# neuronika/neuronika

Measured on NVIDIA H100. Metric: forward+backward GFLOP/s, higher is better.
Workload: dtype bf16

## Files before the change

neuronika_b200/csrc/nk_gemm_tc.cu:

```cuda
#include "nk_internal.cuh"
#include "nk_ptx.cuh"

namespace {

constexpr int BLOCK_M = 128;
constexpr int BLOCK_K = 64;
constexpr int WGMMA_K = 16;
constexpr int kNumThreads = 384;
constexpr uint32_t kSmemLimit = 232448;
constexpr int kEpiCols = 64;
constexpr uint32_t kEpiStageBytes = 2 * 64 * kEpiCols * 4;

struct GemmParams {
  int64_t M, N, K;
  int64_t ldc;
  void* C;
  const void* bias;
  float alpha, beta;
  int bias_bf16;
  int bias_per_row;
  int relu;
  const void* mask;
  float* colsum;
  int num_m_blocks, num_n_blocks, num_k_blocks;
  uint32_t a_lbo, a_sbo, a_kstep;
  uint32_t b_lbo, b_sbo, b_kstep;
  int rs_world, m_rot;
  int64_t rs_rows;
  void* rs_dst[8];
  int batch, a_batched, b_batched, batch_reduce, splits;
  int64_t c_batch_stride;
  int tma_store;
  int64_t bias_batch_stride;
};

__device__ __forceinline__ int tile_m_block(const GemmParams& p, int tile) {
  const int t = tile % p.num_m_blocks;
  if (p.rs_world == 0) return t;
  const int owner = (t + p.m_rot) % p.rs_world;
  return owner * (p.num_m_blocks / p.rs_world) + t / p.rs_world;
}

constexpr int kGroupM = 16;
__device__ __forceinline__ void tile_coords(const GemmParams& p, int tile, int& m_blk, int& n_blk) {
  if (p.rs_world) {
    m_blk = tile_m_block(p, tile);
    n_blk = tile / p.num_m_blocks;
    return;
  }
  const int group_size = kGroupM * p.num_n_blocks;
  const int group = tile / group_size, in_group = tile - group * group_size;
  const int first_m = group * kGroupM;
  const int gm = min(p.num_m_blocks - first_m, kGroupM);
  m_blk = first_m + in_group % gm;
  n_blk = in_group / gm;
}

template <int BLOCK_N>
struct Cfg {
  static constexpr uint32_t A_BYTES = BLOCK_M * BLOCK_K * 2;
  static constexpr uint32_t B_BYTES = BLOCK_N * BLOCK_K * 2;
  static constexpr uint32_t STAGE_BYTES = A_BYTES + B_BYTES;
  static constexpr int kStagesMax = (kSmemLimit - 2048 - kEpiStageBytes) / STAGE_BYTES;
  static constexpr int kStages = kStagesMax > 8 ? 8 : kStagesMax;
  static constexpr uint32_t SMEM_BYTES = kStages * STAGE_BYTES + 2048 + kEpiStageBytes;
};

__device__ __forceinline__ void scale_and_bias(const GemmParams& p, const void* bias, int64_t row, int64_t col0,
                                               const uint32_t* r, bool full, float* v) {
#pragma unroll
  for (int j = 0; j < 32; ++j) v[j] = __fmul_rn(p.alpha, __uint_as_float(r[j]));
  if (bias && p.bias_per_row) {
    const float b = p.bias_bf16 ? __bfloat162float(static_cast<const __nv_bfloat16*>(bias)[row]) : static_cast<const float*>(bias)[row];
#pragma unroll
    for (int j = 0; j < 32; ++j) v[j] += b;
  } else if (bias) {
    if (full && (reinterpret_cast<uintptr_t>(bias) & 15) == 0) {
      if (p.bias_bf16) {
        const uint4* bp = reinterpret_cast<const uint4*>(static_cast<const __nv_bfloat16*>(bias) + col0);
#pragma unroll
        for (int q = 0; q < 4; ++q) {
          const uint4 w = __ldg(bp + q);
          const uint32_t ww[4] = {w.x, w.y, w.z, w.w};
#pragma unroll
          for (int i = 0; i < 4; ++i) {
            v[q * 8 + 2 * i] += __uint_as_float(ww[i] << 16);
            v[q * 8 + 2 * i + 1] += __uint_as_float(ww[i] & 0xffff0000u);
          }
        }
      } else {
        const float4* bp = reinterpret_cast<const float4*>(static_cast<const float*>(bias) + col0);
#pragma unroll
        for (int q = 0; q < 8; ++q) {
          const float4 w = __ldg(bp + q);
          v[q * 4] += w.x, v[q * 4 + 1] += w.y, v[q * 4 + 2] += w.z, v[q * 4 + 3] += w.w;
        }
      }
    } else {
#pragma unroll
      for (int j = 0; j < 32; ++j)
        if (col0 + j < p.N)
          v[j] += p.bias_bf16 ? __bfloat162float(static_cast<const __nv_bfloat16*>(bias)[col0 + j])
                              : static_cast<const float*>(bias)[col0 + j];
    }
  }
}

template <typename TC>
__device__ __forceinline__ void epilogue_colsum_chunk32(const GemmParams& p, int64_t row, int64_t col0, const uint32_t* r,
                                                        int lane, bool vec_ok) {
  float v[32];
  const bool live = row < p.M;
  const TC* mrow = (p.mask && live) ? static_cast<const TC*>(p.mask) + row * p.ldc + col0 : nullptr;
  const bool full = col0 + 32 <= p.N;
#pragma unroll
  for (int j = 0; j < 32; ++j) v[j] = (live && col0 + j < p.N) ? p.alpha * __uint_as_float(r[j]) : 0.f;
  if (mrow) {
    if (full && vec_ok) {
// ... 56 lines not shown
    constexpr int V = 16 / sizeof(TC);
    if (mrow) {
#pragma unroll
      for (int q = 0; q < 32 / V; ++q) {
        NkVec<TC> mk;
        mk.load(mrow + q * V);
#pragma unroll
        for (int i = 0; i < V; ++i) v[q * V + i] = mk.get(i) > 0.f ? v[q * V + i] : 0.f;
      }
    }
    if (p.beta != 0.f) {
#pragma unroll
      for (int q = 0; q < 32 / V; ++q) {
        NkVec<TC> c;
        c.load(crow + q * V);
#pragma unroll
        for (int i = 0; i < V; ++i) v[q * V + i] += p.beta * c.get(i);
      }
    }
    if (p.relu) {
#pragma unroll
      for (int j = 0; j < 32; ++j) v[j] = v[j] > 0.f ? v[j] : 0.f;
    }
#pragma unroll
    for (int q = 0; q < 32 / V; ++q) {
      NkVec<TC> o;
#pragma unroll
      for (int i = 0; i < V; ++i) o.set(i, v[q * V + i]);
      o.store(crow + q * V);
    }
  } else {
#pragma unroll
    for (int j = 0; j < 32; ++j) {
      if (j < ncols && col0 + j < p.N) {
        float x = v[j];
        if (mrow) x = nk_to_f32<TC>(mrow[j]) > 0.f ? x : 0.f;
        if (p.beta != 0.f) x += p.beta * nk_to_f32<TC>(crow[j]);
        if (p.relu) x = x > 0.f ? x : 0.f;
        crow[j] = nk_from_f32<TC>(x);
      }
    }
  }
}

__device__ __forceinline__ int epi_index(int row, int col) {
  return row * kEpiCols + ((((col >> 2) ^ (row & 7))) << 2) + (col & 3);
}

__device__ __forceinline__ float col_bias(const GemmParams& p, int64_t col) {
  if (col >= p.N) return 0.f;
  return p.bias_bf16 ? __bfloat162float(static_cast<const __nv_bfloat16*>(p.bias)[col]) : static_cast<const float*>(p.bias)[col];
}

__device__ __forceinline__ float epi_value(const GemmParams& p, float acc, float bias) {
  float v = __fmul_rn(p.alpha, acc);
  if (p.bias) v += bias;
  return p.relu ? (v > 0.f ? v : 0.f) : v;
}

template <int BLOCK_N, bool A_MN, bool B_MN, typename TC, bool BATCH = false, bool BATCH_BIAS = false>
__global__ void __launch_bounds__(kNumThreads, 1)
gemm_tc_kernel(const __grid_constant__ CUtensorMap tmap_a, const __grid_constant__ CUtensorMap tmap_b,
               const __grid_constant__ CUtensorMap tmap_c, const GemmParams p) {
  using C_ = Cfg<BLOCK_N>;
  constexpr int kStages = C_::kStages;
  constexpr int kStoreCols = 128 / int(sizeof(TC));
  constexpr bool kTmaStore = !BATCH && BLOCK_N % kStoreCols == 0;
  static_assert(2 * 2 * 64 * 128 <= kEpiStageBytes, "staging buffers");
  extern __shared__ uint8_t smem_raw[];
  const uint32_t smem_base = (ptx::smem_u32(smem_raw) + 1023u) & ~1023u;
  const uint32_t smem_a0 = smem_base;
  const uint32_t smem_b0 = smem_base + kStages * C_::A_BYTES;
  const uint32_t bar_base = smem_base + kStages * C_::STAGE_BYTES;
  auto full_bar = [&](int s) { return bar_base + 8u * s; };
  auto empty_bar = [&](int s) { return bar_base + 8u * (kStages + s); };
  const uint32_t epi_stage = bar_base + 1024;
  float* epi = reinterpret_cast<float*>(smem_raw + (epi_stage - ptx::smem_u32(smem_raw)));

  const int wg = threadIdx.x >> 7;
  const int lane = threadIdx.x & 31;

  if (threadIdx.x == 0) {
    ptx::prefetch_tmap(&tmap_a);
    ptx::prefetch_tmap(&tmap_b);
    if (kTmaStore && p.tma_store) ptx::prefetch_tmap(&tmap_c);
    for (int s = 0; s < kStages; ++s) {
      ptx::mbar_init(full_bar(s), 1);
      ptx::mbar_init(empty_bar(s), 2);
    }
    ptx::fence_barrier_init();
  }
  __syncthreads();

  const int tiles_mn = p.num_m_blocks * p.num_n_blocks;
  const int num_tiles = BATCH ? tiles_mn * (p.batch_reduce ? p.splits : p.batch) : tiles_mn;
  auto batch_range = [&](int outer, int& b0, int& b1) {
    if (!p.batch_reduce) {
      b0 = outer, b1 = outer + 1;
    } else {
      const int per = (p.batch + p.splits - 1) / p.splits;
      b0 = outer * per;
      b1 = min(p.batch, b0 + per);
    }
  };

  if (wg == 0) {
    ptx::setmaxnreg_dec<40>();
    if (threadIdx.x == 0) {
      int stage = 0;
      uint32_t phase = 0;
      for (int tile = blockIdx.x; tile < num_tiles; tile += gridDim.x) {
        int m_blk, n_blk, b0 = 0, b1 = 1;
        tile_coords(p, BATCH ? tile % tiles_mn : tile, m_blk, n_blk);
        if (BATCH) batch_range(tile / tiles_mn, b0, b1);
        const int m0 = m_blk * BLOCK_M, n0 = n_blk * BLOCK_N;
        for (int bb = b0; bb < b1; ++bb)
        for (int kb = 0; kb < p.num_k_blocks; ++kb) {
          ptx::mbar_wait_spin(empty_bar(stage), phase ^ 1u);
          ptx::mbar_expect_tx(full_bar(stage), C_::STAGE_BYTES);
          const int k0 = kb * BLOCK_K;
          const uint32_t sa = smem_a0 + stage * C_::A_BYTES;
          const uint32_t sb = smem_b0 + stage * C_::B_BYTES;
          if (A_MN) {
#pragma unroll
            for (int c = 0; c < BLOCK_M / 64; ++c) {
              if (BATCH && p.a_batched)
                ptx::tma_load_3d(sa + c * (64 * BLOCK_K * 2), &tmap_a, full_bar(stage), m0 + c * 64, k0, bb);
              else
                ptx::tma_load_2d(sa + c * (64 * BLOCK_K * 2), &tmap_a, full_bar(stage), m0 + c * 64, k0);
            }
          } else {
            if (BATCH && p.a_batched)
              ptx::tma_load_3d(sa, &tmap_a, full_bar(stage), k0, m0, bb);
            else
              ptx::tma_load_2d(sa, &tmap_a, full_bar(stage), k0, m0);
          }
          if (B_MN) {
#pragma unroll
            for (int c = 0; c < BLOCK_N / 64; ++c) {
              if (BATCH && p.b_batched)
                ptx::tma_load_3d(sb + c * (64 * BLOCK_K * 2), &tmap_b, full_bar(stage), n0 + c * 64, k0, bb);
              else
                ptx::tma_load_2d(sb + c * (64 * BLOCK_K * 2), &tmap_b, full_bar(stage), n0 + c * 64, k0);
            }
          } else {
            if (BATCH && p.b_batched)
              ptx::tma_load_3d(sb, &tmap_b, full_bar(stage), k0, n0, bb);
            else
              ptx::tma_load_2d(sb, &tmap_b, full_bar(stage), k0, n0);
          }
          if (++stage == kStages) {
            stage = 0;
            phase ^= 1u;
          }
        }
      }
    }
    return;
  }

  ptx::setmaxnreg_inc<232>();
  const int cw = wg - 1;
  const int t = threadIdx.x & 127;
  const int warp = t >> 5;
  const bool vec_ok = ((p.ldc * int64_t(sizeof(TC))) % 16 == 0) && ((reinterpret_cast<uintptr_t>(p.C) & 15) == 0) &&
                      ((reinterpret_cast<uintptr_t>(p.mask) & 15) == 0);
  float* stg = epi + cw * (64 * kEpiCols);
  const uint32_t a_off = uint32_t(cw) * (64 * BLOCK_K * 2);
  float acc[BLOCK_N / 2];
  int stage = 0;
  uint32_t phase = 0;
  uint32_t store_buf = 0;
  for (int tile = blockIdx.x; tile < num_tiles; tile += gridDim.x) {
    int m_blk, n_blk;
    tile_coords(p, BATCH ? tile % tiles_mn : tile, m_blk, n_blk);
    int k_total = p.num_k_blocks;
    if (BATCH) {
      int b0, b1;
      batch_range(tile / tiles_mn, b0, b1);
      k_total *= (b1 - b0);
    }
    int prev_stage = 0;
    for (int kb = 0; kb < k_total; ++kb) {
      ptx::mbar_wait_spin(full_bar(stage), phase);
      const uint64_t adesc = ptx::make_smem_desc_sw128(smem_a0 + stage * C_::A_BYTES + a_off, p.a_lbo, p.a_sbo);
      const uint64_t bdesc = ptx::make_smem_desc_sw128(smem_b0 + stage * C_::B_BYTES, p.b_lbo, p.b_sbo);
      ptx::fence_regs(acc);
      ptx::wgmma_fence();
#pragma unroll
      for (int k = 0; k < BLOCK_K / WGMMA_K; ++k)
        ptx::Wgmma<BLOCK_N>::template mma<int(A_MN), int(B_MN)>(acc, adesc + uint64_t((k * p.a_kstep) >> 4),
                                                                 bdesc + uint64_t((k * p.b_kstep) >> 4), (kb | k) != 0 ? 1u : 0u);
      ptx::wgmma_commit();
      ptx::wgmma_wait<1>();
      ptx::fence_regs(acc);
      if (kb > 0 && t == 0) ptx::mbar_arrive(empty_bar(prev_stage));
      prev_stage = stage;
      if (++stage == kStages) {
        stage = 0;
        phase ^= 1u;
      }
    }
    ptx::wgmma_wait<0>();
    ptx::fence_regs(acc);
    if (t == 0) ptx::mbar_arrive(empty_bar(prev_stage));

    if constexpr (kTmaStore) {
      if (p.tma_store) {
        const int fr = warp * 16 + (lane >> 2);
        const int q = lane & 3;
        const int row0 = m_blk * BLOCK_M + cw * 64;
        const uint32_t stg0 = epi_stage + uint32_t(cw) * (2 * 64 * 128);
#pragma unroll
        for (int ch = 0; ch < BLOCK_N / kStoreCols; ++ch) {
          const uint32_t buf = stg0 + store_buf * (64 * 128);
          if (t == 0) ptx::tma_store_wait_read<1>();
          ptx::named_barrier(1 + cw, 128);
          const int64_t col0 = int64_t(n_blk) * BLOCK_N + ch * kStoreCols;
#pragma unroll
          for (int jj = 0; jj < kStoreCols / 8; ++jj) {
            const int j = (ch * (kStoreCols / 8) + jj) * 4;
            const int64_t col = col0 + jj * 8 + 2 * q;
            float b0 = 0.f, b1 = 0.f;
            if (p.bias) b0 = col_bias(p, col), b1 = col_bias(p, col + 1);
            const float v0 = epi_value(p, acc[j], b0), v1 = epi_value(p, acc[j + 1], b1);
            const float v2 = epi_value(p, acc[j + 2], b0), v3 = epi_value(p, acc[j + 3], b1);
            if constexpr (sizeof(TC) == 2) {
              const uint32_t off = fr * 128 + ((jj ^ (fr & 7)) << 4) + 4 * q;
              const __nv_bfloat162 lo = __floats2bfloat162_rn(v0, v1), hi = __floats2bfloat162_rn(v2, v3);
              ptx::st_shared_b32(buf + off, *reinterpret_cast<const uint32_t*>(&lo));
              ptx::st_shared_b32(buf + off + 8 * 128, *reinterpret_cast<const uint32_t*>(&hi));
            } else {
              const uint32_t off = fr * 128 + (((2 * jj + (q >> 1)) ^ (fr & 7)) << 4) + (q & 1) * 8;
              ptx::st_shared_v2_f32(buf + off, v0, v1);
              ptx::st_shared_v2_f32(buf + off + 8 * 128, v2, v3);
            }
          }
          ptx::fence_proxy_async();
          ptx::named_barrier(1 + cw, 128);
          if (t == 0) {
            if (row0 < p.M && col0 < p.N) ptx::tma_store_2d(&tmap_c, buf, int(col0), row0);
            ptx::tma_store_commit();
          }
          store_buf ^= 1u;
        }
        continue;
      }
    }

    const int64_t c_off = (BATCH && !p.batch_reduce) ? int64_t(tile / tiles_mn) * p.c_batch_stride : 0;
    const bool atomic = BATCH && p.batch_reduce;
    const int fr = warp * 16 + (lane >> 2);
    const int fc = (lane & 3) * 2;
    const int half = warp >> 1;
    const int rloc = (warp & 1) * 32 + lane;
    const int64_t row = int64_t(m_blk) * BLOCK_M + cw * 64 + rloc;
    constexpr int kChunks = (BLOCK_N + kEpiCols - 1) / kEpiCols;
#pragma unroll
    for (int ch = 0; ch < kChunks; ++ch) {
      constexpr int kFullBlocks = kEpiCols / 8;
      ptx::named_barrier(1 + cw, 128);
#pragma unroll
      for (int nb = 0; nb < kFullBlocks; ++nb) {
        if (ch * kFullBlocks + nb < BLOCK_N / 8) {
          const int j = (ch * kFullBlocks + nb) * 4;
          *reinterpret_cast<float2*>(stg + epi_index(fr, nb * 8 + fc)) = make_float2(acc[j], acc[j + 1]);
          *reinterpret_cast<float2*>(stg + epi_index(fr + 8, nb * 8 + fc)) = make_float2(acc[j + 2], acc[j + 3]);
        }
      }
      ptx::named_barrier(1 + cw, 128);
      const int chunk_cols = BLOCK_N - ch * kEpiCols < kEpiCols ? BLOCK_N - ch * kEpiCols : kEpiCols;
      if (!vec_ok && !p.colsum && !p.mask && !p.rs_world) {
        const int64_t col_base = int64_t(n_blk) * BLOCK_N + ch * kEpiCols;
        for (int rr = 0; rr < 16; ++rr) {
          const int srow = warp * 16 + rr;
          const int64_t grow = int64_t(m_blk) * BLOCK_M + cw * 64 + srow;
          if (grow >= p.M) break;
          const void* bias = p.bias;
          if constexpr (BATCH_BIAS) bias = batch_bias<true>(p, c_off);
          float rb = 0.f;
          if (bias && p.bias_per_row)
            rb = p.bias_bf16 ? __bfloat162float(static_cast<const __nv_bfloat16*>(bias)[grow]) : static_cast<const float*>(bias)[grow];
          for (int c = lane; c < chunk_cols; c += 32) {
            const int64_t col = col_base + c;
            if (col >= p.N) break;
            float v = __fmul_rn(p.alpha, stg[epi_index(srow, c)]);
            TC* cp = static_cast<TC*>(p.C) + c_off + grow * p.ldc + col;
            if (atomic) {
              if constexpr (sizeof(TC) == 4) atomicAdd(reinterpret_cast<float*>(cp), v);
              continue;
            }
            if (bias) {
              v += p.bias_per_row ? rb
                                  : (p.bias_bf16 ? __bfloat162float(static_cast<const __nv_bfloat16*>(bias)[col])
                                                 : static_cast<const float*>(bias)[col]);
            }
            if (p.beta != 0.f) v += p.beta * nk_to_f32<TC>(*cp);
            if (p.relu) v = v > 0.f ? v : 0.f;
            *cp = nk_from_f32<TC>(v);
          }
        }
        continue;
      }
      const int ncols = min(32, chunk_cols - half * 32);
      if (ncols > 0) {
        uint32_t r[32];
#pragma unroll
        for (int q = 0; q < 8; ++q) {
          float4 v = make_float4(0.f, 0.f, 0.f, 0.f);
          if (q * 4 < ncols) v = *reinterpret_cast<const float4*>(stg + epi_index(rloc, half * 32 + q * 4));
          r[4 * q] = __float_as_uint(v.x), r[4 * q + 1] = __float_as_uint(v.y);
          r[4 * q + 2] = __float_as_uint(v.z), r[4 * q + 3] = __float_as_uint(v.w);
        }
        const int64_t col0 = int64_t(n_blk) * BLOCK_N + ch * kEpiCols + half * 32;
        if (p.colsum && col0 < p.N) epilogue_colsum_chunk32<TC>(p, row, col0, r, lane, vec_ok);
        if (row < p.M && col0 < p.N) epilogue_store_chunk32<TC, BATCH_BIAS>(p, row, col0, r, ncols, vec_ok, c_off, atomic);
      }
    }
  }
  if (kTmaStore && p.tma_store && t == 0) ptx::tma_store_wait<0>();
}

typedef CUresult (*EncodeTiledFn)(CUtensorMap*, CUtensorMapDataType, cuuint32_t, void*, const cuuint64_t*,
                                  const cuuint64_t*, const cuuint32_t*, const cuuint32_t*, CUtensorMapInterleave,
                                  CUtensorMapSwizzle, CUtensorMapL2promotion, CUtensorMapFloatOOBfill);

int make_tmap_2d(nk_ctx* ctx, CUtensorMap* tm, const void* base, int64_t rows, int64_t cols, int64_t ld,
                 uint32_t box_cols, uint32_t box_rows, int dtype = NK_BF16) {
  if (!ctx->encode_tiled) return nk_set_error(ctx, NK_ERR_CUDA, "cuTensorMapEncodeTiled unavailable");
  cuuint64_t dims[2] = {(cuuint64_t)cols, (cuuint64_t)rows};
  cuuint64_t strides[1] = {(cuuint64_t)ld * nk_dtype_size(dtype)};
  cuuint32_t box[2] = {box_cols, box_rows};
  cuuint32_t estr[2] = {1, 1};
  CUresult r = reinterpret_cast<EncodeTiledFn>(ctx->encode_tiled)(
      tm, dtype == NK_BF16 ? CU_TENSOR_MAP_DATA_TYPE_BFLOAT16 : CU_TENSOR_MAP_DATA_TYPE_FLOAT32, 2,
      const_cast<void*>(base), dims, strides, box, estr,
      CU_TENSOR_MAP_INTERLEAVE_NONE, CU_TENSOR_MAP_SWIZZLE_128B, CU_TENSOR_MAP_L2_PROMOTION_L2_256B,
      CU_TENSOR_MAP_FLOAT_OOB_FILL_NONE);
  if (r != CUDA_SUCCESS)
    return nk_set_error(ctx, NK_ERR_CUDA, "cuTensorMapEncodeTiled failed (%d) rows=%lld cols=%lld ld=%lld", (int)r,
                        (long long)rows, (long long)cols, (long long)ld);
  return NK_OK;
}

template <int BLOCK_N, bool A_MN, bool B_MN, typename TC, bool BATCH = false, bool BATCH_BIAS = false>
int launch_cfg(nk_ctx* ctx, const CUtensorMap& ta, const CUtensorMap& tb, const CUtensorMap& tc, GemmParams& p) {
  using C_ = Cfg<BLOCK_N>;
  auto kern = gemm_tc_kernel<BLOCK_N, A_MN, B_MN, TC, BATCH, BATCH_BIAS>;
  static bool attr_done[64] = {};
  if (!attr_done[ctx->device & 63]) {
    static_assert(C_::SMEM_BYTES <= kSmemLimit, "shared memory budget");
    NK_CUDA(ctx, cudaFuncSetAttribute(kern, cudaFuncAttributeMaxDynamicSharedMemorySize, (int)C_::SMEM_BYTES));
    attr_done[ctx->device & 63] = true;
  }
  p.num_n_blocks = int((p.N + BLOCK_N - 1) / BLOCK_N);
  int num_tiles = p.num_m_blocks * p.num_n_blocks;
  if (BATCH) {
    if (p.batch_reduce) {
      int want = (ctx->sm_count + num_tiles - 1) / num_tiles;
      if (want > p.batch) want = p.batch;
      const int per = (p.batch + want - 1) / want;
      p.splits = (p.batch + per - 1) / per;
      num_tiles *= p.splits;
    } else {
      num_tiles *= p.batch;
    }
  }
  const int units = ctx->sm_count;
  const int waves = (num_tiles + units - 1) / units;
  const int grid = (num_tiles + waves - 1) / waves;
  const size_t smem = C_::SMEM_BYTES;
  if (p.rs_world) {
    if (BLOCK_N != 256 || sizeof(TC) != 4 || p.N % 4 != 0)
// ... 60 lines not shown
  p.K = K;
  p.ldc = ldc;
  p.C = C;
  p.bias = bias;
  p.alpha = alpha;
  p.beta = beta;
  p.bias_bf16 = bias_dtype == NK_BF16;
  p.bias_per_row = 0;
  p.relu = relu;
  p.mask = mask;
  p.colsum = colsum;
  p.batch = 1, p.a_batched = p.b_batched = p.batch_reduce = 0, p.splits = 1, p.c_batch_stride = 0, p.bias_batch_stride = 0;
  p.num_m_blocks = int((M + BLOCK_M - 1) / BLOCK_M);
  p.num_n_blocks = 0;
  p.num_k_blocks = int((K + BLOCK_K - 1) / BLOCK_K);
  p.rs_world = 0;
  p.m_rot = 0;
  p.rs_rows = M;
  for (int i = 0; i < 8; ++i) p.rs_dst[i] = nullptr;
  if (ctx->rs_world > 1) {
    if (M % (int64_t(ctx->rs_world) * BLOCK_M) != 0 || beta != 0.f || c_dtype != NK_F32)
      return nk_set_error(ctx, NK_ERR_INVALID_ARG, "wgmma gemm: reduce-scatter epilogue needs M %% (world*128) == 0, "
                          "beta == 0 and f32 output");
    p.rs_world = ctx->rs_world;
    p.rs_rows = M / ctx->rs_world;
    p.m_rot = ctx->rs_rank;
    for (int i = 0; i < ctx->rs_world; ++i) p.rs_dst[i] = ctx->rs_dst[i];
  }
  p.a_lbo = a_mn ? BLOCK_K * 128 : 16;
  p.a_sbo = 1024;
  p.a_kstep = a_mn ? WGMMA_K * 128 : WGMMA_K * 2;
  p.b_lbo = b_mn ? BLOCK_K * 128 : 16;
  p.b_sbo = 1024;
  p.b_kstep = b_mn ? WGMMA_K * 128 : WGMMA_K * 2;

  CUtensorMap ta, tb;
  int rc;
  if (a_mn)
    rc = make_tmap_2d(ctx, &ta, A, K, M, lda, 64, BLOCK_K);
  else
    rc = make_tmap_2d(ctx, &ta, A, M, K, lda, BLOCK_K, BLOCK_M);
  if (rc) return rc;
  if (b_mn)
    rc = make_tmap_2d(ctx, &tb, B, K, N, ldb, 64, BLOCK_K);
  else
    rc = make_tmap_2d(ctx, &tb, B, N, K, ldb, BLOCK_K, (uint32_t)block_n);
  if (rc) return rc;
  const int64_t c_size = int64_t(nk_dtype_size(c_dtype));
  CUtensorMap tc;
  memset(&tc, 0, sizeof(tc));
  p.tma_store = beta == 0.f && !mask && !colsum && !p.rs_world && (block_n * c_size) % 128 == 0 &&
                (reinterpret_cast<uintptr_t>(C) & 15) == 0 && (ldc * c_size) % 16 == 0 && (N * c_size) % 16 == 0;
  if (p.tma_store) {
    rc = make_tmap_2d(ctx, &tc, C, M, N, ldc, uint32_t(128 / c_size), 64, c_dtype);
    if (rc) return rc;
  }

  static const char* names[2][2][5] = {
      {{"wgmma_nt_128x256", "wgmma_nt_128x128", "wgmma_nt_128x64", "wgmma_nt_128x32", "wgmma_nt_128x16"},
       {"wgmma_nn_128x256", "wgmma_nn_128x128", "wgmma_nn_128x64", "", ""}},
      {{"wgmma_tt_128x256", "wgmma_tt_128x128", "wgmma_tt_128x64", "wgmma_tt_128x32", "wgmma_tt_128x16"},
       {"wgmma_tn_128x256", "wgmma_tn_128x128", "wgmma_tn_128x64", "", ""}}};
  const int bi = block_n == 256 ? 0 : block_n == 128 ? 1 : block_n == 64 ? 2 : block_n == 32 ? 3 : 4;
  ctx->last_gemm_kernel = names[a_mn][b_mn][bi];

#define NK_TC(AM, BM_)                                                              \
  (c_dtype == NK_BF16 ? launch_bn<AM, BM_, __nv_bfloat16>(ctx, block_n, ta, tb, tc, p) \
                      : launch_bn<AM, BM_, float>(ctx, block_n, ta, tb, tc, p))
  if (!a_mn && !b_mn) return NK_TC(false, false);
  if (!a_mn && b_mn) return NK_TC(false, true);
  if (a_mn && !b_mn) return NK_TC(true, false);
  return NK_TC(true, true);
#undef NK_TC
}

static int make_tmap_3d(nk_ctx* ctx, CUtensorMap* tm, const void* base, int64_t rows, int64_t cols, int64_t ld, int64_t batch,
                        int64_t batch_stride, uint32_t box_cols, uint32_t box_rows) {
  if (!ctx->encode_tiled) return nk_set_error(ctx, NK_ERR_CUDA, "cuTensorMapEncodeTiled unavailable");
  cuuint64_t dims[3] = {(cuuint64_t)cols, (cuuint64_t)rows, (cuuint64_t)batch};
  cuuint64_t strides[2] = {(cuuint64_t)ld * 2, (cuuint64_t)batch_stride * 2};
  cuuint32_t box[3] = {box_cols, box_rows, 1};
  cuuint32_t estr[3] = {1, 1, 1};
  CUresult r = reinterpret_cast<EncodeTiledFn>(ctx->encode_tiled)(
      tm, CU_TENSOR_MAP_DATA_TYPE_BFLOAT16, 3, const_cast<void*>(base), dims, strides, box, estr,
      CU_TENSOR_MAP_INTERLEAVE_NONE, CU_TENSOR_MAP_SWIZZLE_128B, CU_TENSOR_MAP_L2_PROMOTION_L2_256B,
      CU_TENSOR_MAP_FLOAT_OOB_FILL_NONE);
  if (r != CUDA_SUCCESS)
    return nk_set_error(ctx, NK_ERR_CUDA, "cuTensorMapEncodeTiled (3-d) failed (%d) rows=%lld cols=%lld ld=%lld batch=%lld stride=%lld",
                        (int)r, (long long)rows, (long long)cols, (long long)ld, (long long)batch, (long long)batch_stride);
  return NK_OK;
}

static int gemm_wgmma_batched(nk_ctx* ctx, int transA, int transB, int64_t M, int64_t N, int64_t K, float alpha, const void* A,
                              int64_t lda, int64_t strideA, const void* B, int64_t ldb, int64_t strideB, float beta, void* C,
                              int64_t ldc, int64_t strideC, int64_t batch, int c_dtype, const void* bias, int bias_dtype,
                              int bias_per_row, int64_t bias_stride, int relu, int reduce) {
  if (!nk_gemm_wgmma_supported(transA, transB, M, N, K, A, lda, B, ldb)) return NK_ERR_UNSUPPORTED;
  if (batch < 1 || batch > (int64_t(1) << 30) || (strideA * 2) % 16 != 0 || (strideB * 2) % 16 != 0) return NK_ERR_UNSUPPORTED;
  if (reduce && c_dtype != NK_F32) return NK_ERR_UNSUPPORTED;
  const bool a_mn = transA != 0, b_mn = transB == 0;
  int block_n = N <= 64 ? 64 : (N <= 128 ? 128 : 256);
  GemmParams p;
  p.M = M, p.N = N, p.K = K, p.ldc = ldc, p.C = C;
  p.bias = bias, p.bias_bf16 = bias_dtype == NK_BF16, p.bias_per_row = bias_per_row;
  p.bias_batch_stride = bias ? bias_stride : 0;
  p.alpha = alpha, p.beta = reduce ? 0.f : beta, p.relu = relu, p.mask = nullptr, p.colsum = nullptr;
  p.num_m_blocks = int((M + BLOCK_M - 1) / BLOCK_M);
  p.num_n_blocks = 0;
  p.num_k_blocks = int((K + BLOCK_K - 1) / BLOCK_K);
  p.rs_world = 0, p.m_rot = 0, p.rs_rows = M;
  for (int i = 0; i < 8; ++i) p.rs_dst[i] = nullptr;
  p.batch = int(batch), p.a_batched = strideA != 0, p.b_batched = strideB != 0, p.batch_reduce = reduce ? 1 : 0, p.splits = 1;
  p.c_batch_stride = strideC;
  p.tma_store = 0;
  p.a_lbo = a_mn ? BLOCK_K * 128 : 16, p.a_sbo = 1024, p.a_kstep = a_mn ? WGMMA_K * 128 : WGMMA_K * 2;
  p.b_lbo = b_mn ? BLOCK_K * 128 : 16, p.b_sbo = 1024, p.b_kstep = b_mn ? WGMMA_K * 128 : WGMMA_K * 2;
  CUtensorMap ta, tb;
  int rc;
  if (p.a_batched)
    rc = a_mn ? make_tmap_3d(ctx, &ta, A, K, M, lda, batch, strideA, 64, BLOCK_K)
              : make_tmap_3d(ctx, &ta, A, M, K, lda, batch, strideA, BLOCK_K, BLOCK_M);
  else
    rc = a_mn ? make_tmap_2d(ctx, &ta, A, K, M, lda, 64, BLOCK_K) : make_tmap_2d(ctx, &ta, A, M, K, lda, BLOCK_K, BLOCK_M);
  if (rc) return rc;
  if (p.b_batched)
    rc = b_mn ? make_tmap_3d(ctx, &tb, B, K, N, ldb, batch, strideB, 64, BLOCK_K)
              : make_tmap_3d(ctx, &tb, B, N, K, ldb, batch, strideB, BLOCK_K, (uint32_t)block_n);
  else
    rc = b_mn ? make_tmap_2d(ctx, &tb, B, K, N, ldb, 64, BLOCK_K) : make_tmap_2d(ctx, &tb, B, N, K, ldb, BLOCK_K, (uint32_t)block_n);
  if (rc) return rc;
  CUtensorMap tc;
  memset(&tc, 0, sizeof(tc));
  ctx->last_gemm_kernel = "wgmma_batched";
  const bool per_batch_bias = p.bias && p.bias_batch_stride && !reduce;
#define NK_TCB(BN, AM, BM_)                                                                                      \
  (per_batch_bias ? (c_dtype == NK_BF16 ? launch_cfg<BN, AM, BM_, __nv_bfloat16, true, true>(ctx, ta, tb, tc, p) \
                                        : launch_cfg<BN, AM, BM_, float, true, true>(ctx, ta, tb, tc, p))        \
                  : (c_dtype == NK_BF16 ? launch_cfg<BN, AM, BM_, __nv_bfloat16, true>(ctx, ta, tb, tc, p)       \
                                        : launch_cfg<BN, AM, BM_, float, true>(ctx, ta, tb, tc, p)))
#define NK_TCB_BN(AM, BM_) (block_n == 256 ? NK_TCB(256, AM, BM_) : block_n == 128 ? NK_TCB(128, AM, BM_) : NK_TCB(64, AM, BM_))
  if (!a_mn && !b_mn) return NK_TCB_BN(false, false);
  if (!a_mn && b_mn) return NK_TCB_BN(false, true);
  if (a_mn && b_mn) return NK_TCB_BN(true, true);
  return nk_set_error(ctx, NK_ERR_UNSUPPORTED, "batched gemm: the TT form is not instantiated");
#undef NK_TCB_BN
#undef NK_TCB
}

int nk_gemm_wgmma_batched(nk_ctx* ctx, int transA, int transB, int64_t M, int64_t N, int64_t K, float alpha, const void* A,
                            int64_t lda, int64_t strideA, const void* B, int64_t ldb, int64_t strideB, void* C, int64_t ldc,
                            int64_t strideC, int64_t batch, int c_dtype, const void* row_bias, int bias_dtype, int relu,
                            int reduce) {
  return gemm_wgmma_batched(ctx, transA, transB, M, N, K, alpha, A, lda, strideA, B, ldb, strideB, 0.f, C, ldc, strideC, batch,
                            c_dtype, row_bias, bias_dtype, 1, 0, relu, reduce);
}

extern "C" {

int nk_gemm_bias_act(nk_ctx* ctx, int transA, int transB, int64_t M, int64_t N, int64_t K, float alpha,
                     const void* A, int64_t lda, const void* B, int64_t ldb, float beta, void* C, int64_t ldc,
                     int ab_dtype, int c_dtype, const void* bias, int bias_dtype, int relu) {
  if (!ctx) return NK_ERR_INVALID_ARG;
  NK_REQUIRE(ctx, nk_dtype_ok(ab_dtype) && nk_dtype_ok(c_dtype), "nk_gemm: bad dtype");
  NK_REQUIRE(ctx, M >= 0 && N >= 0 && K >= 0, "nk_gemm: negative dimension");
  if (M == 0 || N == 0) return NK_OK;
  NK_REQUIRE(ctx, C != nullptr && (K == 0 || (A && B)), "nk_gemm: NULL pointer");
  NK_REQUIRE(ctx, lda >= (transA ? M : K) && ldb >= (transB ? K : N) && ldc >= N,
// ... 101 lines not shown
```

neuronika_b200/csrc/nk_ptx.cuh:

```cuda
#pragma once
#include <cuda.h>
#include <stdint.h>

namespace ptx {

__device__ __forceinline__ uint32_t smem_u32(const void* p) {
  return static_cast<uint32_t>(__cvta_generic_to_shared(p));
}

__device__ __forceinline__ bool elect_one() {
  uint32_t pred = 0;
  asm volatile(
      "{\n\t"
      ".reg .b32 %%rx;\n\t"
      ".reg .pred %%px;\n\t"
      "elect.sync %%rx|%%px, %1;\n\t"
      "@%%px mov.s32 %0, 1;\n\t"
      "}\n"
      : "+r"(pred)
      : "r"(0xFFFFFFFFu));
  return pred != 0;
}

__device__ __forceinline__ void mbar_init(uint32_t bar, uint32_t count) {
// ... 37 lines not shown
      : "memory");
  return ok != 0;
}
__device__ __forceinline__ void mbar_wait_spin(uint32_t bar, uint32_t parity) {
  while (!mbar_try_wait_sleep(bar, parity)) {
  }
}

__device__ __forceinline__ void mbar_wait_relaxed(uint32_t bar, uint32_t parity) {
  if (mbar_try_wait(bar, parity)) return;
  uint32_t spins = 0, ns = 32;
  long long t0 = 0;
  while (!mbar_try_wait_sleep(bar, parity)) {
    __nanosleep(ns);
    if (ns < 512) ns <<= 1;
    if ((++spins & 63u) != 0) continue;
    const long long now = clock64();
    if (t0 == 0) t0 = now;
    if (now - t0 > (1ll << 32)) {
      printf("nk_b200: mbarrier watchdog: block %d thread %d bar 0x%x parity %u\n", blockIdx.x, threadIdx.x, bar,
             parity);
      __trap();
    }
  }
}

__device__ __forceinline__ void prefetch_tmap(const CUtensorMap* tmap) {
  asm volatile("prefetch.tensormap [%0];" ::"l"(reinterpret_cast<uint64_t>(tmap)) : "memory");
}
__device__ __forceinline__ void tma_load_2d(uint32_t smem_dst, const CUtensorMap* tmap, uint32_t bar, int32_t c0,
                                            int32_t c1) {
  asm volatile(
      "cp.async.bulk.tensor.2d.shared::cluster.global.mbarrier::complete_tx::bytes [%0], [%1, {%3, %4}], [%2];" ::"r"(
          smem_dst),
      "l"(reinterpret_cast<uint64_t>(tmap)), "r"(bar), "r"(c0), "r"(c1)
      : "memory");
}
__device__ __forceinline__ void tma_load_3d(uint32_t smem_dst, const CUtensorMap* tmap, uint32_t bar, int32_t c0,
                                            int32_t c1, int32_t c2) {
  asm volatile(
      "cp.async.bulk.tensor.3d.shared::cluster.global.mbarrier::complete_tx::bytes [%0], [%1, {%3, %4, %5}], [%2];" ::
          "r"(smem_dst),
      "l"(reinterpret_cast<uint64_t>(tmap)), "r"(bar), "r"(c0), "r"(c1), "r"(c2)
      : "memory");
}
__device__ __forceinline__ void tma_load_4d(uint32_t smem_dst, const CUtensorMap* tmap, uint32_t bar, int32_t c0,
                                            int32_t c1, int32_t c2, int32_t c3) {
  asm volatile(
      "cp.async.bulk.tensor.4d.shared::cluster.global.mbarrier::complete_tx::bytes [%0], [%1, {%3, %4, %5, %6}], "
      "[%2];" ::"r"(smem_dst),
      "l"(reinterpret_cast<uint64_t>(tmap)), "r"(bar), "r"(c0), "r"(c1), "r"(c2), "r"(c3)
      : "memory");
}
__device__ __forceinline__ void tma_store_2d(const CUtensorMap* tmap, uint32_t smem_src, int32_t c0, int32_t c1) {
  asm volatile("cp.async.bulk.tensor.2d.global.shared::cta.bulk_group [%0, {%2, %3}], [%1];" ::"l"(
                   reinterpret_cast<uint64_t>(tmap)),
               "r"(smem_src), "r"(c0), "r"(c1)
               : "memory");
}
__device__ __forceinline__ void tma_store_4d(const CUtensorMap* tmap, uint32_t smem_src, int32_t c0, int32_t c1,
                                             int32_t c2, int32_t c3) {
  asm volatile("cp.async.bulk.tensor.4d.global.shared::cta.bulk_group [%0, {%2, %3, %4, %5}], [%1];" ::"l"(
                   reinterpret_cast<uint64_t>(tmap)),
               "r"(smem_src), "r"(c0), "r"(c1), "r"(c2), "r"(c3)
               : "memory");
}
__device__ __forceinline__ void tma_store_commit() { asm volatile("cp.async.bulk.commit_group;" ::: "memory"); }
__device__ __forceinline__ void st_shared_b32(uint32_t addr, uint32_t v) {
  asm volatile("st.shared.b32 [%0], %1;" ::"r"(addr), "r"(v) : "memory");
}
__device__ __forceinline__ void st_shared_v2_f32(uint32_t addr, float x, float y) {
  asm volatile("st.shared.v2.f32 [%0], {%1, %2};" ::"r"(addr), "f"(x), "f"(y) : "memory");
}
template <int N>
__device__ __forceinline__ void tma_store_wait_read() {
  asm volatile("cp.async.bulk.wait_group.read %0;" ::"n"(N) : "memory");
}
template <int N>
__device__ __forceinline__ void tma_store_wait() {
  asm volatile("cp.async.bulk.wait_group %0;" ::"n"(N) : "memory");
}


template <uint32_t R>
__device__ __forceinline__ void setmaxnreg_dec() { asm volatile("setmaxnreg.dec.sync.aligned.u32 %0;" ::"n"(R)); }
template <uint32_t R>
__device__ __forceinline__ void setmaxnreg_inc() { asm volatile("setmaxnreg.inc.sync.aligned.u32 %0;" ::"n"(R)); }
__device__ __forceinline__ void named_barrier(uint32_t id, uint32_t count) {
  asm volatile("bar.sync %0, %1;" ::"r"(id), "r"(count) : "memory");
}

__device__ __forceinline__ void wgmma_fence() { asm volatile("wgmma.fence.sync.aligned;" ::: "memory"); }
__device__ __forceinline__ void wgmma_commit() { asm volatile("wgmma.commit_group.sync.aligned;" ::: "memory"); }
template <int N>
__device__ __forceinline__ void wgmma_wait() {
  asm volatile("wgmma.wait_group.sync.aligned %0;" ::"n"(N) : "memory");
}
template <int R>
__device__ __forceinline__ void fence_regs(float (&d)[R]) {
#pragma unroll
  for (int i = 0; i < R; ++i) asm volatile("" : "+f"(d[i])::"memory");
}

__device__ __forceinline__ uint64_t make_smem_desc_sw128(uint32_t smem_addr, uint32_t lbo_bytes, uint32_t sbo_bytes) {
  uint64_t d = 0;
  d |= uint64_t((smem_addr >> 4) & 0x3FFFu);
  d |= uint64_t((lbo_bytes >> 4) & 0x3FFFu) << 16;
  d |= uint64_t((sbo_bytes >> 4) & 0x3FFFu) << 32;
  d |= uint64_t(1) << 62;
  return d;
}

template <int N>
struct Wgmma;
template <>
struct Wgmma<16> {
  template <int TA, int TB>
  __device__ __forceinline__ static void mma(float (&d)[8], uint64_t da, uint64_t db, uint32_t scale_d) {
    asm volatile(
        "{\n\t.reg .pred p;\n\tsetp.ne.b32 p, %10, 0;\n\t"
        "wgmma.mma_async.sync.aligned.m64n16k16.f32.bf16.bf16 "
        "{"
        "%0, %1, %2, %3, %4, %5, %6, %7"
        "}, %8, %9, p, 1, 1, %11, %12;\n\t}\n"
        : "+f"(d[0]), "+f"(d[1]), "+f"(d[2]), "+f"(d[3]), "+f"(d[4]), "+f"(d[5]), "+f"(d[6]), "+f"(d[7])
// ... 99 lines not shown
```

Baseline: 744,200.

## Stage bias via bulk copy, per-warp TMA stores with stmatrix epilogue

The producer now bulk-loads the bf16 bias slice for each tile into a double-buffered shared-memory slot alongside the first K stage, guarded by new bias-empty barriers. The epilogue then reads bias from shared memory instead of global memory. Each warp now writes its own 16-row slab with stmatrix and issues its own 16-row TMA store, which replaces the 128-thread named barriers with __syncwarp. The aim is to cut epilogue latency and synchronisation. In exchange it uses 1 KB more shared memory, which may reduce the pipeline stage count, and issues more, smaller TMA stores.

```diff
diff --git a/neuronika_b200/csrc/nk_gemm_tc.cu b/neuronika_b200/csrc/nk_gemm_tc.cu
--- a/neuronika_b200/csrc/nk_gemm_tc.cu
+++ b/neuronika_b200/csrc/nk_gemm_tc.cu
@@ -31,6 +31,7 @@
   int batch, a_batched, b_batched, batch_reduce, splits;
   int64_t c_batch_stride;
   int tma_store;
+  int bias_stage;
   int64_t bias_batch_stride;
 };
 
@@ -61,9 +62,10 @@
   static constexpr uint32_t A_BYTES = BLOCK_M * BLOCK_K * 2;
   static constexpr uint32_t B_BYTES = BLOCK_N * BLOCK_K * 2;
   static constexpr uint32_t STAGE_BYTES = A_BYTES + B_BYTES;
-  static constexpr int kStagesMax = (kSmemLimit - 2048 - kEpiStageBytes) / STAGE_BYTES;
+  static constexpr int kStagesMax = (kSmemLimit - 3072 - kEpiStageBytes) / STAGE_BYTES;
   static constexpr int kStages = kStagesMax > 8 ? 8 : kStagesMax;
-  static constexpr uint32_t SMEM_BYTES = kStages * STAGE_BYTES + 2048 + kEpiStageBytes;
+  static constexpr uint32_t SMEM_BYTES = kStages * STAGE_BYTES + 3072 + kEpiStageBytes;
+  static_assert(2 * BLOCK_N * 2 <= 1024, "bias slots");
 };
 
 __device__ __forceinline__ void scale_and_bias(const GemmParams& p, const void* bias, int64_t row, int64_t col0,
@@ -226,10 +228,67 @@
   return p.bias_bf16 ? __bfloat162float(static_cast<const __nv_bfloat16*>(p.bias)[col]) : static_cast<const float*>(p.bias)[col];
 }
 
+template <bool kAddBias>
 __device__ __forceinline__ float epi_value(const GemmParams& p, float acc, float bias) {
   float v = __fmul_rn(p.alpha, acc);
-  if (p.bias) v += bias;
+  if (kAddBias) v += bias;
   return p.relu ? (v > 0.f ? v : 0.f) : v;
+}
+
+enum { kBiasNone, kBiasStaged, kBiasLoaded };
+
+template <int BLOCK_N, typename TC, int kBias>
+__device__ __forceinline__ void tma_store_tile(const GemmParams& p, const CUtensorMap* tmap_c, const float (&acc)[BLOCK_N / 2],
+                                               int lane, int row0, int64_t n0, uint32_t stg0, uint32_t bias_s,
+                                               uint32_t& store_buf) {
+  constexpr int kStoreCols = 128 / int(sizeof(TC));
+  const int r = lane >> 2;
+  const int q = lane & 3;
+  const int sm_row = (lane & 7) + ((lane >> 3) & 1) * 8;
+  const int sm_blk = lane >> 4;
+#pragma unroll
+  for (int ch = 0; ch < BLOCK_N / kStoreCols; ++ch) {
+    const uint32_t buf = stg0 + store_buf * (64 * 128);
+    if (lane == 0) ptx::tma_store_wait_read<1>();
+    __syncwarp();
+    const int64_t col0 = n0 + ch * kStoreCols;
+    uint32_t packed[4];
+#pragma unroll
+    for (int jj = 0; jj < kStoreCols / 8; ++jj) {
+      const int j = (ch * (kStoreCols / 8) + jj) * 4;
+      float b0 = 0.f, b1 = 0.f;
+      if constexpr (kBias == kBiasStaged) {
+        const uint32_t w = ptx::ld_shared_b32(bias_s + uint32_t(ch * kStoreCols + jj * 8 + 2 * q) * 2);
+        b0 = __uint_as_float(w << 16), b1 = __uint_as_float(w & 0xffff0000u);
+      } else if constexpr (kBias == kBiasLoaded) {
+        const int64_t col = col0 + jj * 8 + 2 * q;
+        b0 = col_bias(p, col), b1 = col_bias(p, col + 1);
+      }
+      constexpr bool kAdd = kBias != kBiasNone;
+      const float v0 = epi_value<kAdd>(p, acc[j], b0), v1 = epi_value<kAdd>(p, acc[j + 1], b1);
+      const float v2 = epi_value<kAdd>(p, acc[j + 2], b0), v3 = epi_value<kAdd>(p, acc[j + 3], b1);
+      if constexpr (sizeof(TC) == 2) {
+        const __nv_bfloat162 lo = __floats2bfloat162_rn(v0, v1), hi = __floats2bfloat162_rn(v2, v3);
+        packed[2 * (jj & 1)] = *reinterpret_cast<const uint32_t*>(&lo);
+        packed[2 * (jj & 1) + 1] = *reinterpret_cast<const uint32_t*>(&hi);
+        if (jj & 1) {
+          const uint32_t off = sm_row * 128 + (((jj - 1 + sm_blk) ^ (sm_row & 7)) << 4);
+          ptx::stmatrix_x4(buf + off, packed[0], packed[1], packed[2], packed[3]);
+        }
+      } else {
+        const uint32_t off = r * 128 + (((2 * jj + (q >> 1)) ^ r) << 4) + (q & 1) * 8;
+        ptx::st_shared_v2_f32(buf + off, v0, v1);
+        ptx::st_shared_v2_f32(buf + off + 8 * 128, v2, v3);
+      }
+    }
+    ptx::fence_proxy_async();
+    __syncwarp();
+    if (lane == 0) {
+      if (row0 < p.M && col0 < p.N) ptx::tma_store_2d(tmap_c, buf, int(col0), row0);
+      ptx::tma_store_commit();
+    }
+    store_buf ^= 1u;
+  }
 }
 
 template <int BLOCK_N, bool A_MN, bool B_MN, typename TC, bool BATCH = false, bool BATCH_BIAS = false>
@@ -248,8 +307,11 @@
   const uint32_t bar_base = smem_base + kStages * C_::STAGE_BYTES;
   auto full_bar = [&](int s) { return bar_base + 8u * s; };
   auto empty_bar = [&](int s) { return bar_base + 8u * (kStages + s); };
+  auto bias_empty_bar = [&](int s) { return bar_base + 8u * (2 * kStages + s); };
   const uint32_t epi_stage = bar_base + 1024;
   float* epi = reinterpret_cast<float*>(smem_raw + (epi_stage - ptx::smem_u32(smem_raw)));
+  auto bias_slot = [&](int s) { return epi_stage + kEpiStageBytes + uint32_t(s) * (BLOCK_N * 2); };
+  const bool stage_bias = kTmaStore && p.tma_store && p.bias_stage;
 
   const int wg = threadIdx.x >> 7;
   const int lane = threadIdx.x & 31;
@@ -262,6 +324,7 @@
       ptx::mbar_init(full_bar(s), 1);
       ptx::mbar_init(empty_bar(s), 2);
     }
+    for (int s = 0; s < 2; ++s) ptx::mbar_init(bias_empty_bar(s), 8);
     ptx::fence_barrier_init();
   }
   __syncthreads();
@@ -283,7 +346,7 @@
     if (threadIdx.x == 0) {
       int stage = 0;
       uint32_t phase = 0;
-      for (int tile = blockIdx.x; tile < num_tiles; tile += gridDim.x) {
+      for (int tile = blockIdx.x, local = 0; tile < num_tiles; tile += gridDim.x, ++local) {
         int m_blk, n_blk, b0 = 0, b1 = 1;
         tile_coords(p, BATCH ? tile % tiles_mn : tile, m_blk, n_blk);
         if (BATCH) batch_range(tile / tiles_mn, b0, b1);
@@ -291,7 +354,15 @@
         for (int bb = b0; bb < b1; ++bb)
         for (int kb = 0; kb < p.num_k_blocks; ++kb) {
           ptx::mbar_wait_spin(empty_bar(stage), phase ^ 1u);
-          ptx::mbar_expect_tx(full_bar(stage), C_::STAGE_BYTES);
+          if (stage_bias && kb == 0) {
+            const int s = local & 1;
+            const uint32_t bytes = 2u * uint32_t(min(int64_t(BLOCK_N), p.N - n0));
+            ptx::mbar_wait_spin(bias_empty_bar(s), ((local >> 1) & 1) ^ 1u);
+            ptx::mbar_expect_tx(full_bar(stage), C_::STAGE_BYTES + bytes);
+            ptx::bulk_load(bias_slot(s), static_cast<const __nv_bfloat16*>(p.bias) + n0, bytes, full_bar(stage));
+          } else {
+            ptx::mbar_expect_tx(full_bar(stage), C_::STAGE_BYTES);
+          }
           const int k0 = kb * BLOCK_K;
           const uint32_t sa = smem_a0 + stage * C_::A_BYTES;
           const uint32_t sb = smem_b0 + stage * C_::B_BYTES;
@@ -345,7 +416,7 @@
   int stage = 0;
   uint32_t phase = 0;
   uint32_t store_buf = 0;
-  for (int tile = blockIdx.x; tile < num_tiles; tile += gridDim.x) {
+  for (int tile = blockIdx.x, local = 0; tile < num_tiles; tile += gridDim.x, ++local) {
     int m_blk, n_blk;
     tile_coords(p, BATCH ? tile % tiles_mn : tile, m_blk, n_blk);
     int k_total = p.num_k_blocks;
@@ -381,42 +452,19 @@
 
     if constexpr (kTmaStore) {
       if (p.tma_store) {
-        const int fr = warp * 16 + (lane >> 2);
-        const int q = lane & 3;
-        const int row0 = m_blk * BLOCK_M + cw * 64;
-        const uint32_t stg0 = epi_stage + uint32_t(cw) * (2 * 64 * 128);
-#pragma unroll
-        for (int ch = 0; ch < BLOCK_N / kStoreCols; ++ch) {
-          const uint32_t buf = stg0 + store_buf * (64 * 128);
-          if (t == 0) ptx::tma_store_wait_read<1>();
-          ptx::named_barrier(1 + cw, 128);
-          const int64_t col0 = int64_t(n_blk) * BLOCK_N + ch * kStoreCols;
-#pragma unroll
-          for (int jj = 0; jj < kStoreCols / 8; ++jj) {
-            const int j = (ch * (kStoreCols / 8) + jj) * 4;
-            const int64_t col = col0 + jj * 8 + 2 * q;
-            float b0 = 0.f, b1 = 0.f;
-            if (p.bias) b0 = col_bias(p, col), b1 = col_bias(p, col + 1);
-            const float v0 = epi_value(p, acc[j], b0), v1 = epi_value(p, acc[j + 1], b1);
-            const float v2 = epi_value(p, acc[j + 2], b0), v3 = epi_value(p, acc[j + 3], b1);
-            if constexpr (sizeof(TC) == 2) {
-              const uint32_t off = fr * 128 + ((jj ^ (fr & 7)) << 4) + 4 * q;
-              const __nv_bfloat162 lo = __floats2bfloat162_rn(v0, v1), hi = __floats2bfloat162_rn(v2, v3);
-              ptx::st_shared_b32(buf + off, *reinterpret_cast<const uint32_t*>(&lo));
-              ptx::st_shared_b32(buf + off + 8 * 128, *reinterpret_cast<const uint32_t*>(&hi));
-            } else {
-              const uint32_t off = fr * 128 + (((2 * jj + (q >> 1)) ^ (fr & 7)) << 4) + (q & 1) * 8;
-              ptx::st_shared_v2_f32(buf + off, v0, v1);
-              ptx::st_shared_v2_f32(buf + off + 8 * 128, v2, v3);
-            }
-          }
-          ptx::fence_proxy_async();
-          ptx::named_barrier(1 + cw, 128);
-          if (t == 0) {
-            if (row0 < p.M && col0 < p.N) ptx::tma_store_2d(&tmap_c, buf, int(col0), row0);
-            ptx::tma_store_commit();
-          }
-          store_buf ^= 1u;
+        const int row0 = m_blk * BLOCK_M + cw * 64 + warp * 16;
+        const int64_t n0 = int64_t(n_blk) * BLOCK_N;
+        const uint32_t stg0 = epi_stage + uint32_t(cw) * (2 * 64 * 128) + uint32_t(warp) * (16 * 128);
+        const uint32_t bias_s = bias_slot(local & 1);
+        if (stage_bias)
+          tma_store_tile<BLOCK_N, TC, kBiasStaged>(p, &tmap_c, acc, lane, row0, n0, stg0, bias_s, store_buf);
+        else if (p.bias)
+          tma_store_tile<BLOCK_N, TC, kBiasLoaded>(p, &tmap_c, acc, lane, row0, n0, stg0, bias_s, store_buf);
+        else
+          tma_store_tile<BLOCK_N, TC, kBiasNone>(p, &tmap_c, acc, lane, row0, n0, stg0, bias_s, store_buf);
+        if (stage_bias) {
+          __syncwarp();
+          if (lane == 0) ptx::mbar_arrive(bias_empty_bar(local & 1));
         }
         continue;
       }
@@ -492,7 +540,7 @@
       }
     }
   }
-  if (kTmaStore && p.tma_store && t == 0) ptx::tma_store_wait<0>();
+  if (kTmaStore && p.tma_store && lane == 0) ptx::tma_store_wait<0>();
 }
 
 typedef CUresult (*EncodeTiledFn)(CUtensorMap*, CUtensorMapDataType, cuuint32_t, void*, const cuuint64_t*,
@@ -659,9 +707,10 @@
   p.tma_store = beta == 0.f && !mask && !colsum && !p.rs_world && (block_n * c_size) % 128 == 0 &&
                 (reinterpret_cast<uintptr_t>(C) & 15) == 0 && (ldc * c_size) % 16 == 0 && (N * c_size) % 16 == 0;
   if (p.tma_store) {
-    rc = make_tmap_2d(ctx, &tc, C, M, N, ldc, uint32_t(128 / c_size), 64, c_dtype);
+    rc = make_tmap_2d(ctx, &tc, C, M, N, ldc, uint32_t(128 / c_size), 16, c_dtype);
     if (rc) return rc;
   }
+  p.bias_stage = p.tma_store && bias && bias_dtype == NK_BF16 && (reinterpret_cast<uintptr_t>(bias) & 15) == 0 && N % 8 == 0;
 
   static const char* names[2][2][5] = {
       {{"wgmma_nt_128x256", "wgmma_nt_128x128", "wgmma_nt_128x64", "wgmma_nt_128x32", "wgmma_nt_128x16"},
@@ -720,6 +769,7 @@
   p.batch = int(batch), p.a_batched = strideA != 0, p.b_batched = strideB != 0, p.batch_reduce = reduce ? 1 : 0, p.splits = 1;
   p.c_batch_stride = strideC;
   p.tma_store = 0;
+  p.bias_stage = 0;
   p.a_lbo = a_mn ? BLOCK_K * 128 : 16, p.a_sbo = 1024, p.a_kstep = a_mn ? WGMMA_K * 128 : WGMMA_K * 2;
   p.b_lbo = b_mn ? BLOCK_K * 128 : 16, p.b_sbo = 1024, p.b_kstep = b_mn ? WGMMA_K * 128 : WGMMA_K * 2;
   CUtensorMap ta, tb;
diff --git a/neuronika_b200/csrc/nk_ptx.cuh b/neuronika_b200/csrc/nk_ptx.cuh
--- a/neuronika_b200/csrc/nk_ptx.cuh
+++ b/neuronika_b200/csrc/nk_ptx.cuh
@@ -113,6 +113,11 @@
       "l"(reinterpret_cast<uint64_t>(tmap)), "r"(bar), "r"(c0), "r"(c1), "r"(c2), "r"(c3)
       : "memory");
 }
+__device__ __forceinline__ void bulk_load(uint32_t smem_dst, const void* src, uint32_t bytes, uint32_t bar) {
+  asm volatile("cp.async.bulk.shared::cluster.global.mbarrier::complete_tx::bytes [%0], [%1], %2, [%3];" ::"r"(smem_dst),
+               "l"(__cvta_generic_to_global(src)), "r"(bytes), "r"(bar)
+               : "memory");
+}
 __device__ __forceinline__ void tma_store_2d(const CUtensorMap* tmap, uint32_t smem_src, int32_t c0, int32_t c1) {
   asm volatile("cp.async.bulk.tensor.2d.global.shared::cta.bulk_group [%0, {%2, %3}], [%1];" ::"l"(
                    reinterpret_cast<uint64_t>(tmap)),
@@ -132,6 +137,16 @@
 }
 __device__ __forceinline__ void st_shared_v2_f32(uint32_t addr, float x, float y) {
   asm volatile("st.shared.v2.f32 [%0], {%1, %2};" ::"r"(addr), "f"(x), "f"(y) : "memory");
+}
+__device__ __forceinline__ uint32_t ld_shared_b32(uint32_t addr) {
+  uint32_t v;
+  asm volatile("ld.shared.b32 %0, [%1];" : "=r"(v) : "r"(addr) : "memory");
+  return v;
+}
+__device__ __forceinline__ void stmatrix_x4(uint32_t addr, uint32_t r0, uint32_t r1, uint32_t r2, uint32_t r3) {
+  asm volatile("stmatrix.sync.aligned.m8n8.x4.shared.b16 [%0], {%1, %2, %3, %4};" ::"r"(addr), "r"(r0), "r"(r1), "r"(r2),
+               "r"(r3)
+               : "memory");
 }
 template <int N>
 __device__ __forceinline__ void tma_store_wait_read() {
```

After: 775,400, median of 6. +4.2%, better.
